# IanMadlenya/pyconsensus

Hardware: AMD Instinct MI355X
Metric: oracle rounds/sec (batched 50x20, 1 GPU) (higher is better)
Workload: dtype f64; 1 GPU; C3: 65536 independent 50x20 oracle rounds per GPU per step (one wavefront per round), inputs resident in HBM, every output of the result dict written (original and filled included); rounds_per_gpu=65536, reporters=50, events=20, parallelism=rounds sharded across 1 GPU(s), no collective

## Files before the change

### pyconsensus_amd/csrc/pcx_batched.hip

```cpp
#include <hip/hip_runtime.h>
#include <stdint.h>
#include <stdlib.h>

#include <type_traits>

#include "pcx_internal.h"

namespace pcx {

namespace {

constexpr int W = 64;
constexpr int NMAX = 64;
constexpr int EMAX = 32;
static_assert(EMAX <= 2 * 16, "2 x 2 grid of 16 x 16 MFMA tiles");
static_assert(NMAX == W, "one reporter per lane");
constexpr int PACKED_WAVES = 4;

constexpr double PI_TOL = 1e-14;
constexpr int PI_MAXIT = 256;
constexpr int PI_PRESQUARE = 3;
constexpr int PI_SQUARE_EVERY = 32;
constexpr int PI_MAX_SQUARINGS = 8;
constexpr int PI_POLISH = 2;
// ... 681 lines not shown
        }
        r = (double)lt + (double)(eq + 1) * 0.5;
        if (__builtin_isnan(x)) r = __builtin_nan("");
    }
    r0 = r;
    r1 = bpermute_d(l + E, r);
    r2 = bpermute_d(l + 2 * E, r);
}

struct Smem {
    double* F;
    double* C;
    double* M;
    double* rep;
    double* n1;
    double* n2;
    double* smooth;
    double* mu;
    double* tot;
    double* guess;
    double* x;
    double* ld;
    double* old;
    double* nv1;
    double* nv2;
    double* adj;
    uint64_t* miss;
};

__host__ __device__ inline int smem_rows(int N) { return (N + 1) & ~1; }
__host__ __device__ inline int cert_stride(int N, int ES) { return (ES & 1) ? (N | 1) : N; }
__host__ __device__ inline int smem_f_size(int N, int E, int ES) {
    return N * ES > E * cert_stride(N, ES) ? N * ES : E * cert_stride(N, ES);
}
__host__ __device__ inline int smem_evs(int E) { return (E + 1) & ~1; }
__host__ __device__ inline int smem_mat(int E, int ES, bool pk) { return pk ? E * (E + 1) / 2 : E * ES; }
__host__ __device__ inline int smem_c_size(int N, int E, int ES, bool pk) {
    if (pk) return smem_rows(N) + 2 * smem_evs(E);
    const int need = 3 * smem_rows(N) + 2 * smem_evs(E);
    return smem_mat(E, ES, pk) > need ? smem_mat(E, ES, pk) : need;
}
__host__ __device__ inline int smem_m_size(int N, int E, int ES, int NR, bool pk) {
    const int scr = med_scr(NR) + smem_evs(E);
    if (pk) {
        const int vec = 2 * smem_rows(N) + 2 * smem_evs(E);
        const int rest = smem_mat(E, ES, pk) - smem_c_size(N, E, ES, pk);
        const int need = scr > vec ? scr : vec;
        return need > rest ? need : rest;
    }
    const int need = scr > 2 * smem_evs(E) ? scr : 2 * smem_evs(E);
    return smem_mat(E, ES, pk) > need ? smem_mat(E, ES, pk) : need;
}

__host__ __device__ inline size_t smem_doubles(int N, int E, int ES, int NR, bool pk) {
    return (size_t)smem_f_size(N, E, ES) + smem_c_size(N, E, ES, pk) + smem_m_size(N, E, ES, NR, pk) +
           (pk ? 1 : 4) * (size_t)smem_evs(E);
}

template <bool PK>
__device__ __forceinline__ int sym_at(int j, int k, int ES) {
    if constexpr (PK)
        return j >= k ? j * (j + 1) / 2 + k : k * (k + 1) / 2 + j;
    else
        return j * ES + k;
}

__device__ Smem carve(double* base, int N, int E, int ES, int NR, bool pk) {
    const int nr = smem_rows(N), ne = smem_evs(E);
    Smem s;
    double* p = base;
    s.F = p; p += smem_f_size(N, E, ES);
    s.C = p; p += smem_c_size(N, E, ES, pk);
    s.M = p; p += smem_m_size(N, E, ES, NR, pk);
    s.miss = reinterpret_cast<uint64_t*>(p); p += ne;
    s.mu = s.x = s.ld = nullptr;
    if (!pk) {
        s.mu = p; p += ne;
        s.x = p; p += ne;
        s.ld = p; p += ne;
    }
    s.tot = s.M + med_scr(NR);
    s.rep = s.C + ne;
    s.guess = s.C;
    if (pk) {
        s.smooth = s.C;
        s.adj = s.C + nr;
        s.old = s.C + nr + ne;
        s.n1 = s.M;
        s.n2 = s.M + nr;
        s.nv1 = s.M + 2 * nr;
        s.nv2 = s.M + 2 * nr + ne;
    } else {
        s.n1 = s.C;
        s.n2 = s.C + nr;
        s.smooth = s.C + 2 * nr;
        s.adj = s.C + 3 * nr;
        s.old = s.C + 3 * nr + ne;
        s.nv1 = s.M;
        s.nv2 = s.M + ne;
    }
    return s;
}

struct RowSpread {
    double lo, hi;
};
__device__ __forceinline__ double pack_d(uint32_t lo, uint32_t hi) {
    return __longlong_as_double((long long)(((uint64_t)hi << 32) | lo));
}
__device__ __forceinline__ void dpp_ready(RowSpread& s) { asm("s_nop 1" : "+v"(s.lo), "+v"(s.hi)); }
__device__ __forceinline__ RowSpread row_spread2(double v) {
    const uint64_t u = (uint64_t)__double_as_longlong(v);
    const auto a = __builtin_amdgcn_permlane16_swap((uint32_t)u, (uint32_t)u, false, false);
    const auto b = __builtin_amdgcn_permlane16_swap((uint32_t)(u >> 32), (uint32_t)(u >> 32), false, false);
    RowSpread s = {pack_d(a[0], b[0]), pack_d(a[1], b[1])};
    dpp_ready(s);
    return s;
}
__device__ __forceinline__ RowSpread row_spread4(double v) {
    const uint64_t u = (uint64_t)__double_as_longlong(v);
    const auto a = __builtin_amdgcn_permlane16_swap((uint32_t)u, (uint32_t)u, false, false);
    const auto b = __builtin_amdgcn_permlane16_swap((uint32_t)(u >> 32), (uint32_t)(u >> 32), false, false);
    const uint32_t ll = __builtin_amdgcn_permlane32_swap(a[0], a[0], false, false)[0];
    const uint32_t lh = __builtin_amdgcn_permlane32_swap(b[0], b[0], false, false)[0];
    const uint32_t hl = __builtin_amdgcn_permlane32_swap(a[1], a[1], false, false)[0];
    const uint32_t hh = __builtin_amdgcn_permlane32_swap(b[1], b[1], false, false)[0];
    RowSpread s = {pack_d(ll, lh), pack_d(hl, hh)};
    dpp_ready(s);
    return s;
}
template <int K, bool NEG = false>
__device__ __forceinline__ void fmac_rowbcast(double& acc, const RowSpread& s, double m) {
    static_assert(K >= 0 && K < 32, "a column of a two-row vector");
    if constexpr (NEG)
        asm("v_fmac_f64_dpp %0, -%1, %2 row_newbcast:%3 row_mask:0xf bank_mask:0xf"
            : "+v"(acc)
            : "v"(K < 16 ? s.lo : s.hi), "v"(m), "n"(K & 15));
    else
        asm("v_fmac_f64_dpp %0, %1, %2 row_newbcast:%3 row_mask:0xf bank_mask:0xf"
            : "+v"(acc)
            : "v"(K < 16 ? s.lo : s.hi), "v"(m), "n"(K & 15));
}
template <int K>
__device__ __forceinline__ double sub_rowbcast(double f, const RowSpread& s, double one) {
    fmac_rowbcast<K, true>(f, s, one);
    return f;
}
template <int K, int ET, class F>
__device__ __forceinline__ void static_cols(F&& f) {
    if constexpr (K < ET) {
        f(std::integral_constant<int, K>());
        static_cols<K + 1, ET>(f);
    }
}

typedef const __attribute__((address_space(3))) double* LdsDoubles;
struct SymBase {
    uint32_t tri, row;
};
__device__ __forceinline__ SymBase sym_base(const double* M, int r) {
    const uint32_t m = (uint32_t)(uintptr_t)(LdsDoubles)M;
    SymBase b = {m + (uint32_t)(r * (r + 1) / 2 * 8), m + (uint32_t)(r * 8)};
    asm("" : "+v"(b.tri), "+v"(b.row));
    return b;
}
template <bool PK, int K>
__device__ __forceinline__ double sym_col(const double* M, const SymBase& b, int r, int ES) {
    if constexpr (!PK) return M[r * ES + K];
    const uint32_t at = K <= r ? b.tri : b.row + 8u * (K * (K + 1) / 2 - K);
    return ((LdsDoubles)(uintptr_t)at)[K];
}

template <bool PK, int ROWS = 4, int ET = 0>
__device__ PCX_OUTLINE double matvec_unit(const double* M, int ES, double xv, int E, const SymBase& sb) {
    const int l = lane_id(), r = l < E ? l : 0;
    double acc = 0.0;
    if constexpr (ET > 0 && ET <= 32) {
        const RowSpread x = row_spread2(xv);
        static_cols<0, ET>([&](auto k) { fmac_rowbcast<k.value>(acc, x, sym_col<PK, k.value>(M, sb, r, ES)); });
    } else {
        for (int k = 0; k < E; k++) acc = fma(M[sym_at<PK>(r, k, ES)], lane_value(xv, k), acc);
    }
    const double y = l < E ? acc : 0.0;
    const double nrm = sqrt(tree_sum<ROWS>(l < E ? y * y : 0.0));
    return l < E ? y / nrm : 0.0;
}

typedef double d4v __attribute__((ext_vector_type(4)));

__device__ __forceinline__ d4v mfma_f64(double a, double b, d4v c) {
    return __builtin_amdgcn_mfma_f64_16x16x4f64(a, b, c, 0, 0, 0);
}

template <bool PK>
__device__ PCX_OUTLINE void square_scaled(double* M, int ES, int E) {
    const int l = lane_id(), ml = l & 15, kq = l >> 4;
    const bool two = E > 16;
    d4v t00 = {0, 0, 0, 0}, t01 = {0, 0, 0, 0}, t10 = {0, 0, 0, 0}, t11 = {0, 0, 0, 0};
    for (int m0 = 0; m0 < E; m0 += 4) {
        const int mm = m0 + kq;
        const bool ok = mm < E;
        const double a0 = (ok && ml < E) ? M[sym_at<PK>(ml, mm, ES)] : 0.0;
        const double b0 = a0;
        t00 = mfma_f64(a0, b0, t00);
        if (two) {
            const double a1 = (ok && 16 + ml < E) ? M[sym_at<PK>(16 + ml, mm, ES)] : 0.0;
            const double b1 = a1;
            if (!PK) t01 = mfma_f64(a0, b1, t01);
            t10 = mfma_f64(a1, b0, t10);
            t11 = mfma_f64(a1, b1, t11);
        }
    }
    double mx = 0.0;
#pragma unroll
    for (int r = 0; r < 4; r++) {
        const int j0 = kq + 4 * r, j1 = 16 + kq + 4 * r, k0 = ml, k1 = 16 + ml;
        if (j0 < E && k0 < E) mx = fmax(mx, fabs(t00[r]));
        if (!PK && j0 < E && k1 < E) mx = fmax(mx, fabs(t01[r]));
        if (j1 < E && k0 < E) mx = fmax(mx, fabs(t10[r]));
        if (j1 < E && k1 < E) mx = fmax(mx, fabs(t11[r]));
    }
    mx = wave_max(mx);
    const bool pow2 = mx >= DBL_MIN_ && __builtin_isfinite(mx);
    const double sc = pow2 ? ldexp(1.0, -ilogb(mx)) : 1.0;
    auto scaled = [&](double t) { return pow2 ? t * sc : (mx > 0.0 ? t / mx : t); };
    wsync();
#pragma unroll
    for (int r = 0; r < 4; r++) {
        const int j0 = kq + 4 * r, j1 = 16 + kq + 4 * r, k0 = ml, k1 = 16 + ml;
        if (j0 < E && k0 < E && (!PK || k0 <= j0)) M[sym_at<PK>(j0, k0, ES)] = scaled(t00[r]);
        if (j0 < E && k1 < E && !PK) M[sym_at<PK>(j0, k1, ES)] = scaled(t01[r]);
        if (j1 < E && k0 < E) M[sym_at<PK>(j1, k0, ES)] = scaled(t10[r]);
        if (j1 < E && k1 < E && (!PK || k1 <= j1)) M[sym_at<PK>(j1, k1, ES)] = scaled(t11[r]);
    }
    wsync();
}

template <int NS>
struct SymOps {
    double a0[NS], a1[NS];
};

template <int NS>
__device__ __forceinline__ void load_sym_ops(const double* C, int E, SymOps<NS>& m) {
    const int l = lane_id(), ml = l & 15, kq = l >> 4;
    const bool two = E > 16;
#pragma unroll
    for (int s = 0; s < NS; s++) {
        m.a0[s] = 0.0;
        m.a1[s] = 0.0;
        if (4 * s < E) {
            const int mm = 4 * s + kq;
            const bool ok = mm < E;
            if (ok && ml < E) m.a0[s] = C[sym_at<true>(ml, mm, 0)];
            if (two && ok && 16 + ml < E) m.a1[s] = C[sym_at<true>(16 + ml, mm, 0)];
        }
    }
}

template <int NS>
__device__ __forceinline__ void store_sym_ops(double* C, int E, const SymOps<NS>& m) {
    const int l = lane_id(), ml = l & 15, kq = l >> 4;
    const bool two = E > 16;
    wsync();
#pragma unroll
    for (int s = 0; s < NS; s++) {
        if (4 * s < E) {
            const int mm = 4 * s + kq;
            if (mm <= ml && ml < E) C[sym_at<true>(ml, mm, 0)] = m.a0[s];
            if (two && mm <= 16 + ml && 16 + ml < E) C[sym_at<true>(16 + ml, mm, 0)] = m.a1[s];
        }
    }
    wsync();
}

template <int NS>
__device__ PCX_OUTLINE void square_scaled_reg(SymOps<NS>& m, int E) {
    const int l = lane_id(), ml = l & 15, kq = l >> 4;
    const bool two = E > 16;
    const bool t01_moves = E <= 20;
    d4v t00 = {0, 0, 0, 0}, t01 = {0, 0, 0, 0}, t10 = {0, 0, 0, 0}, t11 = {0, 0, 0, 0};
#pragma unroll
    for (int s = 0; s < NS; s++) {
        if (4 * s < E) {
            t00 = mfma_f64(m.a0[s], m.a0[s], t00);
            if (two) {
                if (!t01_moves) t01 = mfma_f64(m.a0[s], m.a1[s], t01);
                t10 = mfma_f64(m.a1[s], m.a0[s], t10);
                t11 = mfma_f64(m.a1[s], m.a1[s], t11);
            }
        }
    }
    double mx = 0.0;
#pragma unroll
    for (int r = 0; r < 4; r++) {
        const int j0 = kq + 4 * r, j1 = 16 + kq + 4 * r, k0 = ml, k1 = 16 + ml;
        if (j0 < E && k0 < E) mx = fmax(mx, fabs(t00[r]));
        if (j1 < E && k0 < E) mx = fmax(mx, fabs(t10[r]));
        if (j1 < E && k1 < E) mx = fmax(mx, fabs(t11[r]));
    }
    mx = wave_max(mx);
    const bool pow2 = mx >= DBL_MIN_ && __builtin_isfinite(mx);
    const double sc = pow2 ? ldexp(1.0, -ilogb(mx)) : 1.0;
    auto keep = [&](auto scaled) {
#pragma unroll
        for (int r = 0; r < 4; r++) {
// ... 552 lines not shown
```

### pyconsensus_amd/csrc/pcx_batched_round.inc

```
#if PCX_ROUND_RAGGED >= 2
#define PCX_ROUND_CELL0 rcell
#define PCX_ROUND_ROW0 rrow
#define PCX_ROUND_EV0 rev
#define PCX_ROUND_B rround
template <int NT, int ET, bool CLUS, bool PK>
#if PCX_ROUND_RAGGED == 3
__global__ void __launch_bounds__(64, 3) ragged_kmeans_round_kernel(BatchArgs ka, const MediumDesc* __restrict__ rag,
                                                                    const RoundParams* __restrict__ ptab,
                                                                    const KmeansEntry* __restrict__ ktab) {
#else
__global__ void __launch_bounds__(64, 3) ragged_params_round_kernel(BatchArgs ka, const MediumDesc* __restrict__ rag,
                                                                    const RoundParams* __restrict__ ptab) {
#endif
    static_assert(NT == 0 && ET == 0, "a ragged launch has no compiled shape");
    extern __shared__ __attribute__((aligned(16))) double smem[];
    const MediumDesc* const rd = rag + blockIdx.x;
    const int N = __builtin_amdgcn_readfirstlane(rd->N), E = __builtin_amdgcn_readfirstlane(rd->E), ES = E | 1;
    const int64_t rcell = uniform64(rd->cell), rrow = uniform64(rd->row), rev = uniform64(rd->ev);
    const int64_t rround = __builtin_amdgcn_readfirstlane(rd->round);
    const RoundParams* const rp = ptab + __builtin_amdgcn_readfirstlane(rd->param);
    BatchArgs a = ka;
    a.algorithm = __builtin_amdgcn_readfirstlane(rp->algorithm);
    a.max_components = __builtin_amdgcn_readfirstlane(rp->max_components);
    a.catch_tol = uniform_f64(rp->catch_tol);
    a.alpha = uniform_f64(rp->alpha);
    a.variance_threshold = uniform_f64(rp->variance_threshold);
    a.hierarchy_threshold = uniform_f64(rp->hierarchy_threshold);
    a.cluster_threshold = uniform_f64(rp->cluster_threshold);
#if PCX_ROUND_RAGGED == 3
    const KmeansEntry* const ke = ktab + rround;
    a.kmeans_k = __builtin_amdgcn_readfirstlane(ke->k);
    a.kmeans_init = ka.kmeans_init + uniform64(ke->offset);
#endif
#elif PCX_ROUND_RAGGED
#define PCX_ROUND_CELL0 rcell
#define PCX_ROUND_ROW0 rrow
#define PCX_ROUND_EV0 rev
#define PCX_ROUND_B blockIdx.x
template <int NT, int ET, bool CLUS, bool PK>
__global__ void __launch_bounds__(64, 3) ragged_round_kernel(BatchArgs a, const RaggedDesc* __restrict__ rag) {
    static_assert(NT == 0 && ET == 0, "a ragged launch has no compiled shape");
    extern __shared__ __attribute__((aligned(16))) double smem[];
    const RaggedDesc* const rd = rag + blockIdx.x;
    const int N = __builtin_amdgcn_readfirstlane(rd->N), E = __builtin_amdgcn_readfirstlane(rd->E), ES = E | 1;
    const int64_t rcell = uniform64(rd->cell), rrow = uniform64(rd->row), rev = uniform64(rd->ev);
#else
#define PCX_ROUND_CELL0 (b * (int64_t)N * E)
#define PCX_ROUND_ROW0 (b * N)
#define PCX_ROUND_EV0 (b * E)
#define PCX_ROUND_B blockIdx.x
template <int NT, int ET, bool CLUS, bool PK>
__global__ void __launch_bounds__(64, (NT > 0 && PK) ? PACKED_WAVES : 3) batched_round_kernel(BatchArgs a) {
    extern __shared__ __attribute__((aligned(16))) double smem[];
    const int N = NT > 0 ? NT : a.N, E = ET > 0 ? ET : a.E, ES = ET > 0 ? compiled_es(ET) : a.ES;
#endif
    const int l = lane_id();
    const int64_t b = PCX_ROUND_B;
    constexpr int NRM = NT > 0 ? NT : 64;
    Smem S = carve(smem, N, E, ES, NRM, PK);
    const bool row = l < N, col = l < E;
    const int64_t bo = a.bounds_shared ? 0 : PCX_ROUND_EV0;
    const bool has_bounds = a.scaled != nullptr;
    auto pw_rows = [&](double v) { return wave_pw_sum_lds<NT>(v, N, S.M); };
    auto pw_rows2 = [&](double v1, double v2, double& s1, double& s2) { wave_pw_sum2_lds<NT>(v1, v2, N, S.M, s1, s2); };
    auto pw_cols = [&](double v) { return wave_pw_sum_dpp<ET>(v, E); };
    constexpr int CR = live_rows(ET);

    typedef const __attribute__((address_space(4))) BatchArgs* KernArgs;
    auto out_args = [&]() -> KernArgs {
        uint64_t p = (uint64_t)__builtin_amdgcn_kernarg_segment_ptr();
        asm volatile("" : "+s"(p));
        return (KernArgs)p;
    };

    long long mprof[3] = {0, 0, 0};
    STAMP(0);
    const double* Rg = a.reports + PCX_ROUND_CELL0;
    bool scj = false;
    double loj = 0.0, hij = 0.0;
    if (col && has_bounds) {
        scj = a.scaled[bo + l] != 0;
        loj = a.lo[bo + l];
        hij = a.hi[bo + l];
    }
    double raw = row && a.reputation ? a.reputation[PCX_ROUND_ROW0 + l] : 0.0;
    if constexpr (NT > 0 && ET > 0 && (NT * ET) % 2 == 0) {
        constexpr int TOT2 = NT * ET / 2, NV = (TOT2 + W - 1) / W;
        double2 v[NV];
#pragma unroll
        for (int q = 0; q < NV; q++)
            if (l + W * q < TOT2) v[q] = reinterpret_cast<const double2*>(Rg)[l + W * q];
#pragma unroll
        for (int q = 0; q < NV; q++) {
            const int idx = 2 * (l + W * q);
            if (idx < NT * ET) {
                const int i0 = idx / ET, j0 = idx - i0 * ET;
                const int i1 = (idx + 1) / ET, j1 = idx + 1 - i1 * ET;
                S.F[i0 * ES + j0] = v[q].x;
                S.F[i1 * ES + j1] = v[q].y;
            }
        }
    } else {
        for (int idx = l; idx < N * E; idx += W) {
            const int i = idx / E, j = idx - i * E;
            S.F[i * ES + j] = Rg[idx];
        }
    }
    const uint64_t scaled_mask = ballot(col && scj);

    double rep;
    if (a.reputation) {
        const double tot = pw_rows(raw);
        rep = raw / tot;
    } else {
        rep = 1.0 / (double)N;
    }
    const double tok = trunc(rep * 1e6);
    if (row) S.rep[l] = rep;
    const double denom = tree_sum(row ? tok : 0.0) - 1.0;
    wsync();

    STAMP(1);
    uint32_t nacnt = 0;
    double xnext = row ? S.F[l * ES] : 1.0;
    uint32_t nanb = 0, zerob = 0;
    int zcol = 0;
#pragma unroll(ET > 0 ? ET : 1)
    for (int j = 0; j < E; j++) {
        const bool sc = (scaled_mask >> j) & 1;
        double x = xnext;
        if (j + 1 < E) xnext = row ? S.F[l * ES + j + 1] : 1.0;
        if (sc) {
            const double lo = bcast(loj, j), hi = bcast(hij, j);
            if (row) {
                x = (x - lo) / (hi - lo);
                if (a.int_dtype) x = trunc(x);
                S.F[l * ES + j] = x;
            }
        }
        const bool xn = __builtin_isnan(x), xz = x == 0.0;
        nanb |= xn ? 1u << j : 0u;
        zerob |= xz ? 1u << j : 0u;
        const uint64_t zm = ballot(xz), mm = ballot(xn) | zm;
        zcol = l == j ? popc(zm) : zcol;
        if (l == 0) S.miss[j] = mm;
        asm volatile("" : "+v"(nanb), "+v"(zerob), "+v"(zcol));
    }
    nacnt = (uint32_t)__popc(zerob) | ((uint32_t)__popc(nanb) << 8) | ((uint32_t)zcol << 16);
    wsync();
    if (double* const og = out_args()->original) round_to_global(og + PCX_ROUND_CELL0, S.F, N, E, ES, NT, ET);

    STAMP(2);
    uint64_t miss_j = 0;
    if (col) miss_j = S.miss[l];
    const bool nonneg = !ballot(row && !(rep >= 0.0));
    const bool binary_fill = col && miss_j && !scj;
    bool tot_exact;
    uint64_t need_bin = 0;
    {
        constexpr bool SPLITC = NT > 0 && ET > 0 && 3 * ET <= W;
        const bool split = SPLITC ? nonneg : (nonneg && 3 * E <= W);
        const bool sums = SPLITC ? nonneg : true;
        tot_exact = SPLITC ? false : !split;
        double tot = 0.0, sp = 0.0, sa = 0.0;
        const int g = split ? (l >= E) + (l >= 2 * E) : 0;
        const bool live = l < (split ? 3 * E : E);
        const int c = live ? l - g * E : 0;
        uint64_t m = ~0ull;
        if (sums) {
            const uint64_t past = N < 64 ? ~0ull << N : 0ull;
            const uint64_t mc = split ? S.miss[c] : miss_j;
            m = live ? ((mc | past) >> g) | ~(~0ull >> g) : ~0ull;
        }
        if constexpr (SPLITC) {
            if (split) {
                constexpr int TS = (NT + 2) / 3;
                const double* const Fp = S.F + g * ES + c;
                const double* const rp = S.rep + g;
                const uint32_t mlo = (uint32_t)m, mhi = (uint32_t)(m >> 32);
#pragma unroll
                for (int t = 0; t < TS; t++) {
                    const bool miss = ((3 * t < 32 ? mlo : mhi) & (1u << ((3 * t) & 31))) != 0;
                    const double r0 = rp[3 * t];
                    const uint64_t fu = (uint64_t)__double_as_longlong(Fp[3 * t * ES]);
                    const uint32_t fh = miss ? 0u : (uint32_t)(fu >> 32);
                    const double re = miss ? 0.0 : r0;
                    const double f = __longlong_as_double((long long)(((uint64_t)fh << 32) | (uint32_t)fu));
                    tot = tot + re;
                    sp = fma(re, f, sp);
                    sa = fma(re, fabs(f), sa);
                }
            }
        } else {
            const int G = split ? 3 : 1;
            const double* const Fc = S.F + c;
            for (int k = 0; k < N; k += G) {
                const bool miss = (m >> k) & 1;
                const int i = g + k;
                const double re = miss ? 0.0 : S.rep[i];
                const double f = miss ? 0.0 : Fc[i * ES];
                tot = tot + re;
                sp = fma(re, f, sp);
                sa = fma(fabs(re), fabs(f), sa);
            }
        }
        if (split) {
            const int l1 = (l + E) & (W - 1), l2 = (l + 2 * E) & (W - 1);
            const double t1 = bpermute_d(l1, tot), t2 = bpermute_d(l2, tot);
            const double p1 = bpermute_d(l1, sp), p2 = bpermute_d(l2, sp);
            const double a1 = bpermute_d(l1, sa), a2 = bpermute_d(l2, sa);
            tot = (tot + t1) + t2;
            sp = (sp + p1) + p2;
            sa = (sa + a1) + a2;
        }
        const double t_lo = 1.5 - a.catch_tol, t_hi = 1.5 + a.catch_tol;
        const double accf = sp / tot, margin = 1e-12 * (sa / tot);
        const bool fast = sums && tot > 0.0 && __builtin_isfinite(accf) && __builtin_isfinite(margin) &&
                          fabs(accf - t_lo) > margin && fabs(accf - t_hi) > margin;
        need_bin = ballot(binary_fill && !fast);
        if (binary_fill && fast) {
            double gs = catch_(accf, a.catch_tol);
            if (a.int_dtype) gs = trunc(gs);
            S.guess[l] = gs;
        }
        if (col && miss_j) S.tot[l] = tot;
    }
    wsync();
    STAMP(13);
    {
        uint64_t todo = ballot(col && scj && miss_j != 0);
        auto pair_of = [&](int j, double& x, double& w, bool& present) {
            const uint64_t mj = S.miss[j];
            present = row && !((mj >> l) & 1);
            const double tot = S.tot[j];
            x = row ? S.F[l * ES + j] : 0.0;
            w = present ? S.rep[l] / tot : 0.0;
        };
        auto finish = [&](int j, double g) {
            if (a.int_dtype) g = trunc(g);
            if (l == 0) S.guess[j] = g;
        };
        constexpr int NRS = NT > 0 ? NT : 64, KP = (NRS + 3) & ~3;
        const uint64_t all_j = todo;
        if (todo && a.reputation && nonneg) {
            uint32_t* const kx = reinterpret_cast<uint32_t*>(S.M);
            float* const wf = reinterpret_cast<float*>(S.M) + KP;
            if (l < KP) wf[l] = row ? (float)rep : 0.f;
            for (uint64_t t = todo; t; t &= t - 1) {
                const int j = __builtin_ctzll(t);
                const uint64_t mj = S.miss[j];
                const bool present = row && !((mj >> l) & 1);
                const double x0 = row ? S.F[l * ES + j] : 0.0;
                double g;
                if (wave_wmedian_screen<NRS>(x0, rep, present, S.tot[j], N, kx, wf, g)) {
                    finish(j, g);
                    todo &= ~(1ull << j);
                }
            }
            wsync();
        }
        if (a.stamps && l == 0) {
            a.stamps[b * 32 + 24] = popc(all_j) - popc(todo);
            a.stamps[b * 32 + 25] = popc(todo);
        }
        const bool replay = need_bin || (todo && !tot_exact);
        if (a.stamps && l == 0) {
            a.stamps[b * 32 + 26] = popc(need_bin);
            a.stamps[b * 32 + 27] = replay;
        }
        if (replay) {
            constexpr int NR = NT > 0 ? NT : 64;
            const double* const Fc = S.F + (col ? l : 0);
            double tot = 0.0;
#pragma unroll 10
            for (int i = 0; i < NR; i++) {
                if (i < N) {
                    const bool miss = (miss_j >> i) & 1;
                    const double re = miss ? 0.0 : S.rep[i];
                    tot = tot + re;
                }
            }
            if (need_bin) {
                double ex = 0.0;
#pragma unroll 10
                for (int i = 0; i < NR; i++) {
                    if (i < N) {
                        const double t = (S.rep[i] / tot) * Fc[i * ES];
                        ex = ((miss_j >> i) & 1) ? ex : ex + t;
                    }
                }
                if ((need_bin >> l) & 1) {
                    double gs = catch_(ex, a.catch_tol);
                    if (a.int_dtype) gs = trunc(gs);
                    S.guess[l] = gs;
                }
            }
            if (col && miss_j) S.tot[l] = tot;
            wsync();
        }
        while (todo) {
            const int j = __builtin_ctzll(todo);
            todo &= todo - 1;
            double x0, w0;
            bool p0;
            pair_of(j, x0, w0, p0);
            finish(j, wave_wmedian_rank<(NT > 0 ? NT : 64)>(x0, w0, p0, N, S.M, a.stamps ? mprof : nullptr));
            wsync();
        }
    }
    wsync();
    STAMP(14);
    if (row) {
        uint64_t mn = S.miss[0];
        double gn = S.guess[0];
        for (int j = 0; j < E; j++) {
            const uint64_t mj = mn;
            const double g = gn;
            if (j + 1 < E) {
                mn = S.miss[j + 1];
                gn = S.guess[j + 1];
            }
            if ((mj >> l) & 1) S.F[l * ES + j] = g;
        }
    }
    wsync();
    if (double* const fg = out_args()->filled) round_to_global(fg + PCX_ROUND_CELL0, S.F, N, E, ES, NT, ET);

    STAMP(3);
    double oldj = col ? ob_vecmat(S.rep, S.F + l, ES, N, E, l) : 0.0;

    double sc_i = 0.0, nc_i = 0.0, ld_j = 0.0;
    int branch = 5, flags = 0, iters = 0, comps = -1;
    const int alg = a.algorithm;
    const bool clus = CLUS && alg >= 5;
    const double rep_sum = pw_rows(rep);
    if (alg == 0 || alg == 2 || alg == 3 || clus) {
        const double den = rep_sum;
        double muj = 0.0;
        if (E == 1) {
            const double p = row ? S.F[l * ES] * rep : 0.0;
            const double acc = pw_rows(p);
            muj = acc / den;
        } else if (col) {
            double acc = S.F[l] * S.rep[0];
            for (int i = 1; i < N; i++) acc = acc + S.F[i * ES + l] * S.rep[i];
            muj = acc / den;
        }
        if constexpr (!PK) {
            wsync();
            if (col) S.mu[l] = muj;
            wsync();
        }

        STAMP(4);
        bool nonzero = false, finite = true;
        {
            constexpr int NR = NT > 0 ? NT : 64;
            const int ml = l & 15, kq = l >> 4;
            const bool two = E > 16;
            const double m0 = __shfl(muj, ml), m1 = __shfl(muj, 16 + ml);
            const double mu0 = ml < E ? m0 : 0.0, mu1 = 16 + ml < E ? m1 : 0.0;
            d4v c00 = {0, 0, 0, 0}, c10 = {0, 0, 0, 0}, c11 = {0, 0, 0, 0};
#pragma unroll
            for (int i0 = 0; i0 < NR; i0 += 4) {
                if (i0 < N) {
                    const int i = i0 + kq;
                    const bool ok = i < N;
                    const double tk = ok ? trunc(S.rep[i] * 1e6) : 0.0;
                    const bool v0 = ok && ml < E, v1 = ok && 16 + ml < E;
                    const double d0 = v0 ? S.F[i * ES + ml] - mu0 : 0.0;
                    const double d1 = v1 ? S.F[i * ES + 16 + ml] - mu1 : 0.0;
                    const double a0 = v0 ? d0 * tk : 0.0, a1 = v1 ? d1 * tk : 0.0;
                    c00 = mfma_f64(a0, d0, c00);
                    if (two) {
                        c10 = mfma_f64(a1, d0, c10);
                        c11 = mfma_f64(a1, d1, c11);
                    }
                }
            }
            auto put = [&](int j, int k, double acc) {
                const double c = acc / denom;
                S.C[sym_at<PK>(j, k, ES)] = c;
                if (!PK) {
                    S.M[sym_at<PK>(j, k, ES)] = c;
                    S.C[k * ES + j] = c;
                    S.M[k * ES + j] = c;
                }
                nonzero |= c != 0.0;
                finite &= __builtin_isfinite(c) != 0;
            };
            if constexpr (PK) wsync();
#pragma unroll
            for (int r = 0; r < 4; r++) {
                const int j0 = kq + 4 * r, j1 = 16 + kq + 4 * r, k0 = ml, k1 = 16 + ml;
                if (j0 < E && k0 <= j0) put(j0, k0, c00[r]);
                if (j1 < E && k0 < E) put(j1, k0, c10[r]);
                if (j1 < E && k1 <= j1) put(j1, k1, c11[r]);
            }
        }
        const bool any_nz = ballot(nonzero) != 0;
        const bool all_fin = ballot(!finite) == 0;
        wsync();

        STAMP(5);
        double xv = 0.0;
        if (!all_fin) {
            xv = col ? 1.0 : 0.0;
            flags |= 2;
        } else if (!any_nz) {
            xv = l == 0 ? 1.0 : 0.0;
            flags |= 1;
        } else {
            const double dg = col ? S.C[sym_at<PK>(l, l, ES)] : -__builtin_inf();
            const double dgmax = wave_max<CR>(dg);
            const int kd = __builtin_ctzll(ballot(col && dg == dgmax));
            double x0 = col ? S.C[sym_at<PK>(l, kd, ES)] : 0.0;
            const double n0 = sqrt(tree_sum<CR>(x0 * x0));
            xv = col ? x0 / n0 : 0.0;
            constexpr int NS = !PK ? 1 : ET > 0 ? (ET + 3) / 4 : EMAX / 4;
            SymOps<NS> mreg, creg;
            if constexpr (PK) {
                load_sym_ops<NS>(S.C, E, mreg);
                creg = mreg;
            }
            auto square = [&](bool in_loop) {
                if constexpr (PK) {
                    if (in_loop) load_sym_ops<NS>(S.C, E, mreg);
                    square_scaled_reg<NS>(mreg, E);
                    if (in_loop) store_sym_ops<NS>(S.C, E, mreg);
                } else {
                    square_scaled<PK>(S.M, ES, E);
                }
            };
            int sqn = 0;
            for (; sqn < PI_PRESQUARE; sqn++) square(false);
            if constexpr (PK) store_sym_ops<NS>(S.C, E, mreg);
            const SymBase sb = sym_base(S.C, col ? l : 0);
            int it = 0, since = 0;
            for (;;) {
                const double y = matvec_unit<PK, CR, ET>(PK ? S.C : S.M, ES, xv, E, sb);
                const bool moved = ballot(col && fabs(y - xv) > PI_TOL) != 0;
                xv = y;
                it++;
                since++;
                if (!moved) break;
                if (it >= PI_MAXIT) {
                    flags |= 4;
                    break;
                }
                if (since >= PI_SQUARE_EVERY && sqn < PI_MAX_SQUARINGS) {
                    square(true);
                    sqn++;
                    since = 0;
                }
            }
            if constexpr (PK) store_sym_ops<NS>(S.C, E, creg);
            for (int p = 0; p < PI_POLISH; p++) xv = matvec_unit<PK, CR, ET>(S.C, ES, xv, E, sb);
            const uint64_t nzm = ballot(col && xv != 0.0);
            if (nzm) {
                const double xf = bcast(xv, __builtin_ctzll(nzm));
                const bool neg = popc(nzm) == 1 ? xf < 0.0 : xf > 0.0;
                if (neg) xv = -xv;
            }
            iters = it + PI_POLISH + sqn;
// ... 126 lines not shown
                d1 = d;
                d2 = __longlong_as_double((long long)(((uint64_t)uhi << 32) | ulo));
            }
        }
        if (col) {
            const double t = 0.01 * oldj;
            S.nv1[l] = d1 + t;
            S.nv2[l] = d2 + t;
        }
        wsync();
        double ref = 0.0;
        if (alg == 0) {
            double r0, r1, r2;
            if (3 * E <= W) {
                rank_avg3(S.old, S.nv1, S.nv2, E, r0, r1, r2);
            } else {
                r0 = rank_avg(S.old, E);
                r1 = rank_avg(S.nv1, E);
                r2 = rank_avg(S.nv2, E);
            }
            const double e1 = fabs(r1 - r0), e2 = fabs(r2 - r0);
            ref = pw_cols(e1) - pw_cols(e2);
        }
        bool pick1;
        if (ref == 0) {
            const double q1 = d1 - oldj, q2 = d2 - oldj;
            const double ref2 = pw_cols(q1 * q1) - pw_cols(q2 * q2);
            pick1 = ref2 <= 0;
            branch = pick1 ? 3 : 4;
        } else {
            pick1 = ref < 0;
            branch = pick1 ? 1 : 2;
        }
        nc_i = pick1 ? set1 : set2;
    }

    STAMP(7);
    const double meanrep = rep_sum / (double)N;
    double u = fabs(nc_i * (rep / meanrep));
    double Su = pw_rows(u);
    const bool rep_masked = alg == 0 && __builtin_isnan(Su);
    if (Su == 0) {
        u += 1.0;
        Su = pw_rows(u);
    }
    const double this_i = u / Su;
    const double smooth_i = a.alpha * this_i + (1.0 - a.alpha) * rep;
    wsync();
    if (row) S.smooth[l] = smooth_i;
    wsync();

    STAMP(8);
    double lo2 = NT > 0 ? 0.0 : loj, hi2 = NT > 0 ? 0.0 : hij;
    if constexpr (NT > 0) {
        if (col && scj) {
            lo2 = a.lo[bo + l];
            hi2 = a.hi[bo + l];
        }
    }
    double rawj = col ? ob_vecmat(S.smooth, S.F + l, ES, N, E, l) : 0.0;
    STAMP(15);
    if (scaled_mask) {
        const double Wt = tree_sum(row ? smooth_i : 0.0);
        const double mid = 0.5 * Wt, slack = 0x1p-45 * Wt;
        const double Mg = 0x1p-44 * Wt + slack + DBL_EPS;
        const bool wok = Mg < __builtin_inf() && !ballot(row && !(smooth_i >= 0.0 && smooth_i < mid - slack)) &&
                         ballot(row && smooth_i > 0.0) != 0;
        uint64_t slow = 0;
        constexpr bool FGSPLIT = NT > 0 && ET > 0 && 3 * ET <= W;
        if constexpr (FGSPLIT) {
            slow = scaled_mask;
            if (wok) {
                constexpr int TS = (NT + 2) / 3;
                const int g = (l >= ET) + (l >= 2 * ET);
                const bool live = l < 3 * ET;
                const int c = live ? l - g * ET : 0;
                const uint64_t mc = S.miss[c];
                const int fm = mc ? __builtin_ctzll(mc) : 0;
                const double gf = S.F[fm * ES + c];
                const double* const Fp = S.F + g * ES + c;
                const double* const wp = S.smooth + g;
                double below = 0.0, group = 0.0;
                bool sawnan = false;
#pragma unroll
                for (int t = 0; t < TS; t++) {
                    const bool in = 3 * t + 2 < NT || g + 3 * t < NT;
                    const double x = Fp[3 * t * ES], w = in ? wp[3 * t] : 0.0;
                    const double ib = in && x < gf ? 1.0 : 0.0, ig = in && x == gf ? 1.0 : 0.0;
                    below = fma(w, ib, below);
                    group = fma(w, ig, group);
                    sawnan |= in && x != x;
                }
                const int l1 = (l + ET) & (W - 1), l2 = (l + 2 * ET) & (W - 1);
                const double b1 = bpermute_d(l1, below), b2 = bpermute_d(l2, below);
                const double g1 = bpermute_d(l1, group), g2 = bpermute_d(l2, group);
                below = (below + b1) + b2;
                group = (group + g1) + g2;
                const uint64_t nm = ballot(live && sawnan);
                const bool cnan = (((nm | (nm >> ET)) | (nm >> (2 * ET))) >> l) & 1;
                const bool decided = col && scj && mc != 0 && gf != 0.0 && fabs(gf) < 0x1p1023 && !cnan &&
                                     below <= mid - Mg && below + group > mid + Mg;
                if (decided) rawj = gf;
                slow = scaled_mask & ~ballot(decided);
            }
        } else
        for (uint64_t todo = scaled_mask; todo; todo &= todo - 1) {
            const int j = __builtin_ctzll(todo);
            const double x0 = row ? S.F[l * ES + j] : 0.0;
            const uint64_t mj = (uint64_t)uniform64((int64_t)S.miss[j]);
            bool decided = false;
            if (wok && mj) {
                const double g = bcast(x0, __builtin_ctzll(mj));
                if (g != 0.0 && fabs(g) < 0x1p1023 && !ballot(row && x0 != x0)) {
                    const double below = tree_sum(row && x0 < g ? smooth_i : 0.0);
                    const double group = tree_sum(row && x0 == g ? smooth_i : 0.0);
                    decided = below <= mid - Mg && below + group > mid + Mg;
                    if (decided && l == j) rawj = g;
                }
            }
            if (!decided) slow |= 1ull << j;
        }
        if (a.stamps && l == 0) {
            a.stamps[b * 32 + 22] = popc(scaled_mask) - popc(slow);
            a.stamps[b * 32 + 23] = popc(slow);
        }
        while (slow) {
            const int j = __builtin_ctzll(slow);
            slow &= slow - 1;
            const double x0 = row ? S.F[l * ES + j] : 0.0;
            const double m = wave_wmedian_rank<(NT > 0 ? NT : 64)>(x0, smooth_i, row, N, S.M, a.stamps ? mprof : nullptr);
            if (l == j) rawj = m;
            wsync();
        }
    }
    STAMP(16);
    double adjj = 0.0, finj = 0.0;
    if (col) {
        if (scj) {
            adjj = rawj;
            finj = adjj * (hi2 - lo2);
            finj = finj + lo2;
        } else {
            adjj = catch_(rawj, a.catch_tol);
            finj = adjj;
        }
        S.adj[l] = adjj;
    }
    wsync();

    STAMP(9);
    double certj = 0.0;
    {
        uint64_t* hitm = reinterpret_cast<uint64_t*>(S.M);
        double fn = row ? S.F[l * ES] : 0.0, an = S.adj[0];
        for (int j = 0; j < E; j++) {
            const double f = fn, av = an;
            if (j + 1 < E) {
                fn = row ? S.F[l * ES + j + 1] : 0.0;
                an = S.adj[j + 1];
            }
            const uint64_t hm = ballot(row && f == av);
            if (l == 0) hitm[j] = hm;
        }
        wsync();
        const int NS = cert_stride(N, ES);
        double* comp = S.F;
        for (int j = 0; j < E; j++) {
            const uint64_t hm = hitm[j];
            if ((hm >> l) & 1) comp[j * NS + mbcnt64(hm)] = smooth_i;
        }
        wsync();
        if (col) {
            constexpr int TMAX = (NT > 0 ? NT : 64) / 8;
            const uint64_t hm = hitm[l];
            const int n = popc(hm), T = n >> 3;
            const double* c = comp + l * NS;
            double res = 0.0;
            if (T) {
                double r[8];
#pragma unroll
                for (int k = 0; k < 8; k++) r[k] = c[k];
#pragma unroll
                for (int t = 1; t < TMAX; t++)
                    if (t < T) {
#pragma unroll
                        for (int k = 0; k < 8; k++) r[k] = r[k] + c[8 * t + k];
                    }
                res = ((r[0] + r[1]) + (r[2] + r[3])) + ((r[4] + r[5]) + (r[6] + r[7]));
            }
            for (int q = 8 * T; q < n; q++) res = res + c[q];
            certj = n ? res : (a.algorithm == 0 ? __builtin_nan("") : 0.0);
        }
    }
    double ac = fabs(certj);
    double Sc = pw_cols(ac);
    if (Sc == 0) {
        ac += 1.0;
        Sc = pw_cols(ac);
    }
    const double reward = ac / Sc;
    const double avg_cert = pw_cols(certj) / (double)E;

    STAMP(10);
    double pcj = 0.0, nzj = 0.0;
    const bool smooth_finite = !ballot(row && !__builtin_isfinite(smooth_i));
    if (col) {
        const uint64_t nam = S.miss[l];
        double s = 0.0, c = 0.0;
        auto step = [&](double x, double y) {
            const double p = x * y;
            const double pe = fma(x, y, -p);
            const double t = s + p;
            const double z = t - s;
            const double se = (s - (t - z)) + (p - z);
            s = t;
            c = c + (pe + se);
        };
        if (smooth_finite) {
            for (uint64_t mm = nam; mm; mm &= mm - 1) step(S.smooth[__builtin_ctzll(mm)], 1.0);
        } else {
            for (int i = 0; i < N; i++) step(S.smooth[i], ((nam >> i) & 1) ? 1.0 : 0.0);
        }
        pcj = 1.0 - (s + c);
        nzj = (double)((nacnt >> 16) & 0xffu);
    }
    double narow = 0.0;
    int nnan = 0;
    if (row) {
        narow = (double)(nacnt & 0xffu);
        nnan = (int)((nacnt >> 8) & 0xffu);
    }
    const bool rowmasked = row && nnan == E;
    const double pr = 1.0 - narow / (double)E;
    const double pna = 1.0 - pw_cols(pcj) / (double)E;
    double ar = rowmasked ? 0.0 : fabs(pr);
    double Sr = pw_rows(ar);
    if (Sr == 0) {
        ar = rowmasked ? 0.0 : fabs(pr) + 1.0;
        Sr = pw_rows(ar);
    }
    const double rel = rowmasked ? fabs(pr) : ar / Sr;
    double apc = fabs(pcj);
    double Spc = pw_cols(apc);
    if (Spc == 0) {
        apc += 1.0;
        Spc = pw_cols(apc);
    }
    const double relc = apc / Spc;

    STAMP(11);
    const auto oa = out_args();
    if (row) {
        const int64_t o = PCX_ROUND_ROW0 + l;
        if (oa->old_rep) oa->old_rep[o] = rep;
        if (oa->this_rep) oa->this_rep[o] = this_i;
        if (oa->smooth_rep) oa->smooth_rep[o] = smooth_i;
        if (oa->scores) oa->scores[o] = sc_i;
        if (oa->na_row) oa->na_row[o] = narow;
        if (oa->participation_rows) oa->participation_rows[o] = pr;
        if (oa->relative_part) oa->relative_part[o] = rel;
        if (oa->reporter_bonus) oa->reporter_bonus[o] = (rowmasked || rep_masked) ? rel : rel * pna + smooth_i * (1.0 - pna);
    }
    if (col) {
        const int64_t o = PCX_ROUND_EV0 + l;
        if (oa->adj_first_loadings) oa->adj_first_loadings[o] = ld_j;
        if (oa->outcomes_raw) oa->outcomes_raw[o] = rawj;
        if (oa->outcomes_adjusted) oa->outcomes_adjusted[o] = adjj;
        if (oa->outcomes_final) oa->outcomes_final[o] = finj;
        if (oa->certainty) oa->certainty[o] = certj;
        if (oa->consensus_reward) oa->consensus_reward[o] = reward;
        if (oa->nas_filled) oa->nas_filled[o] = nzj;
        if (oa->participation_columns) oa->participation_columns[o] = rep_masked ? 1.0 : pcj;
        if (oa->author_bonus) oa->author_bonus[o] = rep_masked ? 1.0 : relc * pna + reward * (1.0 - pna);
    }
    if (l == 0) {
        if (oa->participation) oa->participation[b] = 1.0 - pna;
        if (oa->avg_certainty) oa->avg_certainty[b] = avg_cert;
        if (oa->branch) oa->branch[b] = branch;
        if (oa->flags) oa->flags[b] = flags;
        if (oa->pi_iters) oa->pi_iters[b] = iters;
        if (oa->components) oa->components[b] = comps;
    }
    STAMP(12);
    if (a.stamps && threadIdx.x == 0) {
        a.stamps[b * 32 + 20] = mprof[0];
        a.stamps[b * 32 + 21] = mprof[1];
    }
}
#undef PCX_ROUND_CELL0
#undef PCX_ROUND_ROW0
#undef PCX_ROUND_EV0
#undef PCX_ROUND_B
```

Measured before the change: 73.39 million rounds/s.

## Keep row values and per-column masks in registers for compiled shapes

For compiled shapes, each lane now loads its whole report row into registers with 16-byte LDS reads. Per-column miss and hit masks are gathered into lanes with v_writelane instead of being written to LDS by lane 0 and read back. The same approach is applied to the NaN/zero scan, the fill-in of missing values and the certainty hit-mask pass, which removes serial LDS round trips and one barrier phase. The cost is higher register pressure (an ET-length array per lane), which could reduce occupancy.

```diff
diff --git a/pyconsensus_amd/csrc/pcx_batched.hip b/pyconsensus_amd/csrc/pcx_batched.hip
--- a/pyconsensus_amd/csrc/pcx_batched.hip
+++ b/pyconsensus_amd/csrc/pcx_batched.hip
@@ -857,6 +857,12 @@
         f(std::integral_constant<int, K>());
         static_cols<K + 1, ET>(f);
     }
+}
+template <int K>
+__device__ __forceinline__ uint32_t write_lane(uint32_t v, uint32_t s) {
+    static_assert(K >= 0 && K < W, "a lane of the wave");
+    asm("v_writelane_b32 %0, %1, %2" : "+v"(v) : "s"(__builtin_amdgcn_readfirstlane((int)s)), "n"(K));
+    return v;
 }
 
 typedef const __attribute__((address_space(3))) double* LdsDoubles;
diff --git a/pyconsensus_amd/csrc/pcx_batched_round.inc b/pyconsensus_amd/csrc/pcx_batched_round.inc
--- a/pyconsensus_amd/csrc/pcx_batched_round.inc
+++ b/pyconsensus_amd/csrc/pcx_batched_round.inc
@@ -61,6 +61,8 @@
     const bool row = l < N, col = l < E;
     const int64_t bo = a.bounds_shared ? 0 : PCX_ROUND_EV0;
     const bool has_bounds = a.scaled != nullptr;
+    constexpr bool REPFLAG = NT > 0 && ET > 0;
+    const bool rep_flag = REPFLAG && a.reputation != nullptr;
     auto pw_rows = [&](double v) { return wave_pw_sum_lds<NT>(v, N, S.M); };
     auto pw_rows2 = [&](double v1, double v2, double& s1, double& s2) { wave_pw_sum2_lds<NT>(v1, v2, N, S.M, s1, s2); };
     auto pw_cols = [&](double v) { return wave_pw_sum_dpp<ET>(v, E); };
@@ -83,7 +85,7 @@
         loj = a.lo[bo + l];
         hij = a.hi[bo + l];
     }
-    double raw = row && a.reputation ? a.reputation[PCX_ROUND_ROW0 + l] : 0.0;
+    double raw = row && (REPFLAG ? rep_flag : a.reputation != nullptr) ? a.reputation[PCX_ROUND_ROW0 + l] : 0.0;
     if constexpr (NT > 0 && ET > 0 && (NT * ET) % 2 == 0) {
         constexpr int TOT2 = NT * ET / 2, NV = (TOT2 + W - 1) / W;
         double2 v[NV];
@@ -109,7 +111,7 @@
     const uint64_t scaled_mask = ballot(col && scj);
 
     double rep;
-    if (a.reputation) {
+    if (REPFLAG ? rep_flag : a.reputation != nullptr) {
         const double tot = pw_rows(raw);
         rep = raw / tot;
     } else {
@@ -122,9 +124,51 @@
 
     STAMP(1);
     uint32_t nacnt = 0;
-    double xnext = row ? S.F[l * ES] : 1.0;
     uint32_t nanb = 0, zerob = 0;
     int zcol = 0;
+    constexpr bool ROWREG = NT > 0 && ET > 0;
+    uint32_t missb = 0;
+    uint32_t mjlo = 0, mjhi = 0;
+    if constexpr (ROWREG) {
+        static_assert(compiled_es(ET) % 2 == 0, "16-byte row reads");
+        double xr[ET];
+#pragma unroll
+        for (int j = 0; j < ET; j++) xr[j] = 1.0;
+        if (row) {
+            const double2* const Fr = reinterpret_cast<const double2*>(S.F + l * ES);
+#pragma unroll
+            for (int q = 0; q < ET / 2; q++) {
+                const double2 v = Fr[q];
+                xr[2 * q] = v.x;
+                xr[2 * q + 1] = v.y;
+            }
+            if (ET & 1) xr[ET - 1] = S.F[l * ES + ET - 1];
+        }
+        static_cols<0, ET>([&](auto jc) {
+            constexpr int j = jc.value;
+            const bool sc = (scaled_mask >> j) & 1;
+            double x = xr[j];
+            if (sc) {
+                const double lo = bcast(loj, j), hi = bcast(hij, j);
+                if (row) {
+                    x = (x - lo) / (hi - lo);
+                    if (a.int_dtype) x = trunc(x);
+                    S.F[l * ES + j] = x;
+                }
+            }
+            const bool xn = __builtin_isnan(x), xz = x == 0.0;
+            nanb |= xn ? 1u << j : 0u;
+            zerob |= xz ? 1u << j : 0u;
+            const uint64_t zm = ballot(xz), mm = ballot(xn) | zm;
+            zcol = (int)write_lane<j>((uint32_t)zcol, (uint32_t)popc(zm));
+            mjlo = write_lane<j>(mjlo, (uint32_t)mm);
+            mjhi = write_lane<j>(mjhi, (uint32_t)(mm >> 32));
+            asm volatile("" : "+v"(nanb), "+v"(zerob), "+v"(zcol), "+v"(mjlo), "+v"(mjhi));
+        });
+        missb = nanb | zerob;
+        if (col) S.miss[l] = ((uint64_t)mjhi << 32) | mjlo;
+    } else {
+    double xnext = row ? S.F[l * ES] : 1.0;
 #pragma unroll(ET > 0 ? ET : 1)
     for (int j = 0; j < E; j++) {
         const bool sc = (scaled_mask >> j) & 1;
@@ -146,13 +190,18 @@
         if (l == 0) S.miss[j] = mm;
         asm volatile("" : "+v"(nanb), "+v"(zerob), "+v"(zcol));
     }
+    }
     nacnt = (uint32_t)__popc(zerob) | ((uint32_t)__popc(nanb) << 8) | ((uint32_t)zcol << 16);
     wsync();
     if (double* const og = out_args()->original) round_to_global(og + PCX_ROUND_CELL0, S.F, N, E, ES, NT, ET);
 
     STAMP(2);
     uint64_t miss_j = 0;
-    if (col) miss_j = S.miss[l];
+    if constexpr (ROWREG) {
+        if (col) miss_j = ((uint64_t)mjhi << 32) | mjlo;
+    } else {
+        if (col) miss_j = S.miss[l];
+    }
     const bool nonneg = !ballot(row && !(rep >= 0.0));
     const bool binary_fill = col && miss_j && !scj;
     bool tot_exact;
@@ -242,7 +291,7 @@
         };
         constexpr int NRS = NT > 0 ? NT : 64, KP = (NRS + 3) & ~3;
         const uint64_t all_j = todo;
-        if (todo && a.reputation && nonneg) {
+        if (todo && (REPFLAG ? rep_flag : a.reputation != nullptr) && nonneg) {
             uint32_t* const kx = reinterpret_cast<uint32_t*>(S.M);
             float* const wf = reinterpret_cast<float*>(S.M) + KP;
             if (l < KP) wf[l] = row ? (float)rep : 0.f;
@@ -310,6 +359,16 @@
     }
     wsync();
     STAMP(14);
+    if constexpr (ROWREG) {
+        if (row) {
+            double gs[ET];
+#pragma unroll
+            for (int j = 0; j < ET; j++) gs[j] = S.guess[j];
+#pragma unroll
+            for (int j = 0; j < ET; j++)
+                if ((missb >> j) & 1) S.F[l * ES + j] = gs[j];
+        }
+    } else
     if (row) {
         uint64_t mn = S.miss[0];
         double gn = S.guess[0];
@@ -742,6 +801,36 @@
     double certj = 0.0;
     {
         uint64_t* hitm = reinterpret_cast<uint64_t*>(S.M);
+        const int NS = cert_stride(N, ES);
+        double* comp = S.F;
+        uint64_t hm_l = 0;
+        if constexpr (ROWREG) {
+            double fr[ET];
+#pragma unroll
+            for (int j = 0; j < ET; j++) fr[j] = 0.0;
+            if (row) {
+                const double2* const Fr = reinterpret_cast<const double2*>(S.F + l * ES);
+#pragma unroll
+                for (int q = 0; q < ET / 2; q++) {
+                    const double2 v = Fr[q];
+                    fr[2 * q] = v.x;
+                    fr[2 * q + 1] = v.y;
+                }
+                if (ET & 1) fr[ET - 1] = S.F[l * ES + ET - 1];
+            }
+            wsync();
+            uint32_t hlo = 0, hhi = 0;
+            static_cols<0, ET>([&](auto jc) {
+                constexpr int j = jc.value;
+                const double av = bcast(adjj, j);
+                const uint64_t hm = ballot(row && fr[j] == av);
+                if ((hm >> l) & 1) comp[j * NS + mbcnt64(hm)] = smooth_i;
+                hlo = write_lane<j>(hlo, (uint32_t)hm);
+                hhi = write_lane<j>(hhi, (uint32_t)(hm >> 32));
+            });
+            hm_l = ((uint64_t)hhi << 32) | hlo;
+            wsync();
+        } else {
         double fn = row ? S.F[l * ES] : 0.0, an = S.adj[0];
         for (int j = 0; j < E; j++) {
             const double f = fn, av = an;
@@ -753,16 +842,15 @@
             if (l == 0) hitm[j] = hm;
         }
         wsync();
-        const int NS = cert_stride(N, ES);
-        double* comp = S.F;
         for (int j = 0; j < E; j++) {
             const uint64_t hm = hitm[j];
             if ((hm >> l) & 1) comp[j * NS + mbcnt64(hm)] = smooth_i;
         }
         wsync();
+        }
         if (col) {
             constexpr int TMAX = (NT > 0 ? NT : 64) / 8;
-            const uint64_t hm = hitm[l];
+            const uint64_t hm = ROWREG ? hm_l : hitm[l];
             const int n = popc(hm), T = n >> 3;
             const double* c = comp + l * NS;
             double res = 0.0;
```

Result: faster. 76.27 million rounds/s (median of 6 runs) (+3.9%).
